# lebrice/blurred-GAN

Hardware: AMD Instinct MI355X
Metric: images/sec (G+D+GP step) (higher is better)
Workload: dtype f32; 1 GPU; celeba64 64x64x3 batch 256/GPU, blur sigma 5.0 (31 taps), D-step+GP+G-step+Adam; global_batch=256, parallelism=dp1

## Files before the change

blurred-gan_amd/_lib.py:

```python
from __future__ import annotations

import ctypes as C
import os

HERE = os.path.dirname(os.path.abspath(__file__))
LIB_PATH = os.environ.get("BGAN_HIP_LIB") or os.path.join(HERE, "libbgan_hip.so")


class BgError(RuntimeError):
    pass


class Epilogue(C.Structure):
    _fields_ = [("mode", C.c_int), ("bias", C.c_void_p), ("ref", C.c_void_p), ("keep", C.c_void_p),
                ("alpha", C.c_float), ("scale", C.c_float), ("splitk_ws", C.c_void_p), ("splitk_ws_bytes", C.c_size_t),
                ("keep_elems", C.c_size_t), ("stats", C.c_void_p), ("stats_capacity", C.c_size_t), ("stats_rows", C.POINTER(C.c_int))]


ABI_VERSION = 5
EPI_NONE, EPI_BIAS_LRELU, EPI_MUL_GRAD, EPI_TANH, EPI_AFFINE_LRELU = 0, 1, 2, 3, 4

_p, _i, _f, _z, _u64 = C.c_void_p, C.c_int, C.c_float, C.c_size_t, C.c_uint64

SIGNATURES = {
# ... 4 lines not shown
    "bg_prof_reset": (_i, []),
    "bg_prof_count": (_i, []),
    "bg_prof_get": (_i, [_i, C.c_char_p, _i, C.POINTER(_f), C.POINTER(C.c_double), C.POINTER(C.c_double)]),
    "bg_prof_get_exec": (_i, [_i, C.POINTER(C.c_double)]),
    "bg_prof_get_useful": (_i, [_i, C.POINTER(C.c_double)]),
    "bg_conv2d_useful_flops": (C.c_double, [_i] * 7),
    "bg_range_enable": (_i, [_i]),
    "bg_range_push": (_i, [C.c_char_p]),
    "bg_range_pop": (_i, []),
    "bg_blur_policy": (_i, [_f, _i, _i, C.POINTER(_f), C.POINTER(_f), C.POINTER(_i)]),
    "bg_gauss_kernel_1d": (_i, [_f, _f, C.POINTER(_f), _i, C.POINTER(_i)]),
    "bg_blur_workspace_bytes": (_z, [_i, _i, _i, _i, _i]),
    "bg_blur_nhwc_f32": (_i, [_p, _p, _i, _i, _i, _i, _p, _i, _p, _p]),
    "bg_blur3_lerp_supported": (_i, [_i, _i, _i, _i, _i]),
    "bg_blur3_lerp_nhwc_f32": (_i, [_p, _p, _p, _p, _i, _i, _i, _i, _p, _i, _p]),
    "bg_conv2d_splitk_workspace_bytes": (_z, [_i, _i, _i, _i, _i, _i, _i, _i]),
    "bg_conv2d_fwd": (_i, [_p, _p, _p, _i, _i, _i, _i, _i, _i, _i, C.POINTER(Epilogue), _p]),
    "bg_conv2d_bwd_data": (_i, [_p, _p, _p, _i, _i, _i, _i, _i, _i, _i, C.POINTER(Epilogue), _p]),
    "bg_conv2d_fwd_math": (_i, [_p, _p, _p, _i, _i, _i, _i, _i, _i, _i, C.POINTER(Epilogue), _p, _i]),
    "bg_conv2d_bwd_data_math": (_i, [_p, _p, _p, _i, _i, _i, _i, _i, _i, _i, C.POINTER(Epilogue), _p, _i]),
    "bg_conv2d_math_taken": (_i, [_i] * 9),
    "bg_conv2d_bwd_filter_workspace_bytes": (_z, [_i, _i, _i, _i, _i, _i, _i]),
    "bg_conv2d_bwd_filter": (_i, [_p, _p, _p, _i, _i, _i, _i, _i, _i, _i, _f, _f, _p, _z, _p]),
    "bg_transpose_last2": (_i, [_p, _p, _i, _i, _i, _p]),
    "bg_transpose_last2_batched": (_i, [_p, _p, _p, _i, _i, _p]),
    "bg_gemm_f32": (_i, [_p, _p, _p, _i, _i, _i, _i, _i, _p, _f, _f, _p]),
    "bg_colsum_workspace_bytes": (_z, [_i, _i]),
    "bg_colsum_f32": (_i, [_p, _p, _i, _i, _i, _f, _f, _p, _z, _p]),
    "bg_bn_workspace_bytes": (_z, [_i, _i]),
    "bg_bn_train_fwd": (_i, [_p, _p, _i, _i, _p, _p, _p, _p, _p, _p, _f, _f, _i, _f, _p, _z, _p]),
    "bg_bn_train_fwd_partials": (_i, [_p, _i, _p, _p, _i, _i, _p, _p, _p, _p, _p, _p, _f, _f, _i, _f, _p]),
    "bg_bn_sums_from_partials": (_i, [_p, _i, _i, _p, _p]),
    "bg_bn_infer_fwd": (_i, [_p, _p, _i, _i, _p, _p, _p, _p, _f, _f, _p]),
    "bg_bn_train_bwd": (_i, [_p, _p, _p, _p, _i, _i, _p, _p, _p, _p, _p, _p, _f, _p, _z, _p]),
    "bg_bn_fold_f32": (_i, [_p, _p, _p, _p, _f, _i, _p, _p, _p]),
    "bg_bn_fold_many_f32": (_i, [_i, _p, _p, _p, _p, _p, _p, _p, _p, _p]),
    "bg_bn_stats_f32": (_i, [_p, _i, _i, _p, _p, _z, _p]),
    "bg_bn_finalize_f32": (_i, [_p, _i, _i, _p, _p, _p, _p, _f, _f, _i, _p]),
    "bg_bn_apply_f32": (_i, [_p, _p, _i, _i, _p, _p, _p, _p, _f, _p]),
    "bg_bn_finalize_apply_f32": (_i, [_p, _i, _p, _p, _i, _i, _p, _p, _p, _p, _p, _p, _f, _f, _i, _f, _p]),
    "bg_bn_bwd_stats_f32": (_i, [_p, _p, _p, _i, _i, _p, _p, _p, _p, _f, _p, _p, _z, _p]),
    "bg_bn_bwd_apply_f32": (_i, [_p, _p, _p, _p, _i, _i, _i, _p, _p, _p, _p, _p, _f, _p]),
    "bg_bn_param_grads_f32": (_i, [_p, _i, _f, _p, _p, _p]),
    "bg_lerp_f32": (_i, [_p, _p, _p, _p, _i, _i, _p]),
    "bg_row_norm_f32": (_i, [_p, _p, _i, _i, _p]),
    "bg_gp_seed_f32": (_i, [_p, _p, _f, _p, _i, _i, _p]),
# ... 79 lines not shown
```

blurred-gan_amd/csrc/conv_wgrad.hip:

```cpp
#include "conv_common.h"
#include <algorithm>
#include <cmath>
#include <cstdlib>
#include <mutex>
#include <type_traits>
#include <utility>

namespace {

typedef float floatx16 __attribute__((ext_vector_type(16)));

struct WgradParams {
  const float* X;
  const float* DY;
  float* out;
  int B, H, W, Ci, Ho, Wo, Co;
  int k, s, pt, pl;
  int M;
  int chunk;
  int ksplit;
  int tiles_m, tiles_n, xcd_swizzle;
  float beta, scale;
  unsigned x_bytes, dy_bytes;
  unsigned mul_hw, sh_hw, mul_w, sh_w;
  int lg_w, lg_h, lg_b, pow2;
  int order_n;
  unsigned char tap_order[32];
};

__device__ inline int fastdiv(int m, unsigned mul, unsigned sh) { return (int)(((unsigned long long)(unsigned)m * mul) >> sh); }

template <int BM, int BN, int BKP, int WAVES_M, int WAVES_N, int WAVES_K, int P2>
__global__ __launch_bounds__(256) void conv_wgrad_v3_kernel(const WgradParams p) {
  static_assert(WAVES_M * WAVES_N * WAVES_K == 4, "4 waves");
  constexpr int WTM = BM / WAVES_M, WTN = BN / WAVES_N;
  constexpr int MI = WTM / 32, NI = WTN / 32;
  static_assert(MI >= 1 && NI >= 1 && WTM % 32 == 0 && WTN % 32 == 0, "wave tile");
  constexpr int TPR_A = BM / 4, RPP_A = 256 / TPR_A, AP = BKP / RPP_A;
  constexpr int TPR_B = BN / 4, RPP_B = 256 / TPR_B, BP = BKP / RPP_B;
  static_assert(AP >= 1 && BP >= 1 && BKP % RPP_A == 0 && BKP % RPP_B == 0, "loader passes must tile the chunk exactly");
  constexpr int STAGE = BKP * (BM + BN);
  constexpr int RED = (WAVES_K > 1) ? (WAVES_K - 1) * WAVES_M * WAVES_N * MI * NI * 1024 : 0;
  constexpr int SMEM = (2 * STAGE > RED) ? 2 * STAGE : RED;
  constexpr unsigned kOob = 0x80000000u;
  __shared__ __attribute__((aligned(16))) float smem[SMEM];

  const int tid = threadIdx.x, lane = tid & 63, wave = tid >> 6;
  const int wk = wave % WAVES_K, wmn = wave / WAVES_K;
  const int wm = wmn / WAVES_N, wn = wmn % WAVES_N;
  const int ntile = p.tiles_m * p.tiles_n, ntap = p.k * p.k;
  int tile, tap, zsplit;
  if (P2 == 2 && p.order_n > 0) {
    const int w = blockIdx.x, r = w >> 8;
    const int u = ((r & 1) && ((r + 1) << 8) <= (int)gridDim.x) ? (r << 8) + ((31 - ((w & 255) >> 3)) << 3) + (w & 7) : w;
    tile = u % ntile;
    const int rest = u / ntile;
    zsplit = rest % p.ksplit;
    tap = p.tap_order[rest / p.ksplit];
  } else {
    const int L = p.xcd_swizzle ? bg::xcd_remap(blockIdx.x, gridDim.x) : (int)blockIdx.x;
    tile = L % ntile; tap = (L / ntile) % ntap; zsplit = L / (ntile * ntap);
  }
  const int tile_m = tile / p.tiles_n, tile_n = tile % p.tiles_n;
  const int ci0 = tile_m * BM, co0 = tile_n * BN;
  const int kh = tap / p.k, kw = tap % p.k;
  const int m_begin = zsplit * p.chunk;
  const int m_end = min(p.M, m_begin + p.chunk);
  const int nsteps = (m_end - m_begin + BKP - 1) / BKP;

  const __amdgpu_buffer_rsrc_t rsX = __builtin_amdgcn_make_buffer_rsrc(const_cast<float*>(p.X), 0, (int)p.x_bytes, 0x00020000);
  const __amdgpu_buffer_rsrc_t rsY = __builtin_amdgcn_make_buffer_rsrc(const_cast<float*>(p.DY), 0, (int)p.dy_bytes, 0x00020000);
  const int arow = tid / TPR_A, aq = tid % TPR_A;
  const int brow = tid / TPR_B, bq = tid % TPR_B;
  const int HoWo = p.Ho * p.Wo;
  const bool a_col_ok = ci0 + aq * 4 < p.Ci, b_col_ok = co0 + bq * 4 < p.Co;
  const int a_coloff = (ci0 + aq * 4) * 4, b_coloff = (co0 + bq * 4) * 4;
  const int dyk = kh - p.pt, dxk = kw - p.pl;
  float4 regA[AP], regB[BP];

  const int WoS = p.Wo * p.s, HoS = p.Ho * p.s;
  int dstep_ow, dstep_oh, dstep_b;
// ... 39 lines not shown
      const int bb = r >> (p.lg_w + p.lg_h), oh = (r >> p.lg_w) & (p.Ho - 1), ow = r & (p.Wo - 1);
      t_r[i] = r;
      t_oy[i] = oh * p.s;
      t_ox[i] = ow * p.s;
      t_off[i] = (unsigned)(((bb * p.H + oh * p.s) * p.W + ow * p.s) * p.Ci * 4 + a_coloff);
    }
  }
  if (P2 == 2) {
#pragma unroll
    for (int i = 0; i < AP; ++i) {
      const int r = arow + i * RPP_A;
      t_r[i] = r;
      t_oy[i] = 0;
      t_ox[i] = 0;
      t_off[i] = a_col_ok ? (unsigned)(r * p.H * p.W * p.Ci * 4 + a_coloff) : kOob;
    }
#pragma unroll
    for (int i = 0; i < BP; ++i) b_off[i] = b_col_ok ? (unsigned)((brow + i * RPP_B) * HoWo * p.Co * 4 + b_coloff) : kOob;
  }
  int s_m0 = m_begin;
  int q_oh = 0, q_ow = 0, q_bc = 0, q_left = 0, q_ow_lo = 0, q_ow_hi = 0, q_nb = 1;
  int nsteps_live = 0;
  if (P2 == 2) {
    const int oh_lo = max(0, (-dyk + p.s - 1) / p.s), oh_hi = min(p.Ho - 1, (p.H - 1 - dyk) / p.s);
    const int ow_lo = max(0, (-dxk + p.s - 1) / p.s), ow_hi = min(p.Wo - 1, (p.W - 1 - dxk) / p.s);
    const int rh = max(0, oh_hi - oh_lo + 1), rw = max(0, ow_hi - ow_lo + 1);
    q_nb = p.B / BKP;
    const int nlive = rh * rw * q_nb;
    const int cpz = (nlive + p.ksplit - 1) / p.ksplit;
    const int q_begin = min(nlive, zsplit * cpz), q_end = min(nlive, q_begin + cpz);
    nsteps_live = q_end - q_begin;
    q_left = nsteps_live;
    const int pi = q_begin / q_nb;
    q_bc = q_begin - pi * q_nb;
    q_oh = oh_lo + (rw > 0 ? pi / rw : 0);
    q_ow = ow_lo + (rw > 0 ? pi % rw : 0);
    q_ow_lo = ow_lo; q_ow_hi = ow_hi;
  }

  auto gload = [&](int) {
    if (P2 == 2) {
      if (q_left > 0) {
        const int b0 = q_bc * BKP, pos = q_oh * p.Wo + q_ow;
        const unsigned offS = (unsigned)(((b0 * p.H + q_oh * p.s + dyk) * p.W + q_ow * p.s + dxk) * p.Ci * 4);
        const unsigned offY = (unsigned)((b0 * HoWo + pos) * p.Co * 4);
#pragma unroll
        for (int i = 0; i < AP; ++i)
          regA[i] = __builtin_bit_cast(float4, __builtin_amdgcn_raw_buffer_load_b128(rsX, t_off[i], (int)offS, 0));
#pragma unroll
        for (int i = 0; i < BP; ++i)
          regB[i] = __builtin_bit_cast(float4, __builtin_amdgcn_raw_buffer_load_b128(rsY, b_off[i], (int)offY, 0));
        --q_left;
        if (++q_bc == q_nb) {
// ... 113 lines not shown
    if (wk > 0) {
      float* red = smem + (((wk - 1) * WAVES_M * WAVES_N + wmn) * MI * NI) * 1024;
#pragma unroll
      for (int i = 0; i < MI; ++i)
#pragma unroll
        for (int j = 0; j < NI; ++j)
#pragma unroll
          for (int r = 0; r < 16; ++r) red[((i * NI + j) * 16 + r) * 64 + lane] = acc[i][j][r];
    }
    __syncthreads();
    if (wk > 0) return;
#pragma unroll
    for (int w = 1; w < WAVES_K; ++w) {
      const float* red = smem + (((w - 1) * WAVES_M * WAVES_N + wmn) * MI * NI) * 1024;
#pragma unroll
      for (int i = 0; i < MI; ++i)
#pragma unroll
        for (int j = 0; j < NI; ++j)
#pragma unroll
          for (int r = 0; r < 16; ++r) acc[i][j][r] += red[((i * NI + j) * 16 + r) * 64 + lane];
    }
  }

  float* out = p.out + (size_t)zsplit * p.k * p.k * p.Ci * p.Co + (size_t)tap * p.Ci * p.Co;
  const bool direct = p.ksplit == 1;
#pragma unroll
  for (int i = 0; i < MI; ++i)
#pragma unroll
    for (int j = 0; j < NI; ++j) {
      const int co = co0 + wn * WTN + j * 32 + (lane & 31);
#pragma unroll
      for (int r = 0; r < 16; ++r) {
        const int ci = ci0 + wm * WTM + i * 32 + (r & 3) + 8 * (r >> 2) + 4 * (lane >> 5);
        if (ci < p.Ci && co < p.Co) {
          float* q = out + (size_t)ci * p.Co + co;
          const float v = acc[i][j][r];
          if (direct) *q = (p.beta != 0.f ? p.beta * *q : 0.f) + p.scale * v;
          else *q = v;
        }
      }
    }
}

template <int TG, int BN, int WAVES_N, int WAVES_K>
__global__ __launch_bounds__(256) void conv_wgrad_tg_kernel(const WgradParams p) {
  static_assert(WAVES_N * WAVES_K == 4 && BN == 32 * WAVES_N, "one 32-wide co tile per wave column");
  constexpr int BKP = 32, BMc = 32, BM = TG * BMc;
  constexpr int TPR_B = BN / 4, RPP_B = 256 / TPR_B, BP = BKP / RPP_B;
// ... 1013 lines not shown
      red[zg][c] = make_float4(a.x + b.x, a.y + b.y, a.z + b.z, a.w + b.w);
    }
    __syncthreads();
  }
  if (zg != 0 || e >= n) return;
  const float4 a = red[0][c];
  float4 o = make_float4(scale * a.x, scale * a.y, scale * a.z, scale * a.w);
  if (beta != 0.f) {
    const float4 q = *reinterpret_cast<const float4*>(dw + e);
    o.x += beta * q.x; o.y += beta * q.y; o.z += beta * q.z; o.w += beta * q.w;
  }
  *reinterpret_cast<float4*>(dw + e) = o;
}

__global__ __launch_bounds__(256) void wgrad_reduce_scalar_kernel(const float* __restrict__ slabs, float* __restrict__ dw, int n,
                                                                  int ksplit, float beta, float scale) {
  const int e = blockIdx.x * 256 + threadIdx.x;
  if (e >= n) return;
  float s = 0.f;
  for (int z = 0; z < ksplit; ++z) s += slabs[(size_t)z * n + e];
  dw[e] = (beta != 0.f ? beta * dw[e] : 0.f) + scale * s;
}

struct WgradPlan {
  int mode;
  int ksplit, chunk, tiles_m, tiles_n, bkp, taps_in_grid;
  int always_slab;
};

inline bool strip_ok(int H, int W, int Ci, int Co, int k, int s) {
  if (k != 5 || s != 2 || (H & 1) || (W & 1) || Ci % 32 || Co % 64) return false;
  const int Wo = W / 2, Ho = H / 2;
  if (Wo != 8 && Wo != 16 && Wo != 32) return false;
  return Ho % (64 / Wo) == 0;
}

constexpr size_t kRowLdsMax = 64 * 1024;
inline int thin_ci_rows(int s) { return s == 2 ? 8 : 16; }
inline size_t thin_ci_lds(int W, int Ci, int Co, int k, int s) {
  return std::max((size_t)((thin_ci_rows(s) - 1) * s + k) * ((size_t)W * Ci + 2 * kTiHalo), (size_t)k * (Co / 16) * 4 * 64) * sizeof(float);
}
inline size_t thin_co_lds(int W, int Ci, int Co, int k) {
  return std::max((size_t)(kTcRows + k - 1) * ((size_t)W * Co + 2 * kTcHalo), (size_t)4 * k * (Ci / 16) * 4 * 64) * sizeof(float);
}

WgradPlan plan_wgrad(int B, int H, int W, int Ci, int Co, int k, int s) {
  WgradPlan pl{};
  int Ho, Wo, pt, pp;
  bg::same_pads(H, k, s, &Ho, &pt);
  bg::same_pads(W, k, s, &Wo, &pp);
  const long M = (long)B * Ho * Wo;
  const bool mfma = (Ci % 4 == 0) && (Co % 4 == 0) && Ci >= 16 && Co >= 16;
  const int kk = k * k;
  const bool thin_ci = Ci <= 4 && Co % 4 == 0 && Co >= 16 && kk * Ci <= 128;
  const bool thin_co = Co <= 4 && Ci % 4 == 0 && Ci >= 16 && s == 1 && kk * Co <= 128;
  int bm = 0, bn = 0;
  if (!mfma && !thin_ci && !thin_co) {
    pl.mode = 0;
    const long nblk = bg::cdiv((size_t)k * k * Ci * Co, 256);
    long want = std::max(1L, 2048 / nblk);
    long chunk = std::max(256L, (M + want - 1) / want);
    pl.chunk = (int)chunk;
    pl.ksplit = (int)((M + chunk - 1) / chunk);
    return pl;
  }
  static const int no_strip = getenv("BG_WGRAD_NO_STRIP") ? 1 : 0;
// ... 94 lines not shown
    want = std::max(1L, (tgt + base - 1) / base);
    want = std::min(want, std::max(1L, steps / (skipping ? 8 : 4)));
    if ((size_t)kk * Ci * Co * sizeof(float) > (8u << 20)) want = std::min(want, 2L);
  } else {
    const int bm_eff = pl.taps_in_grid == 2 ? k * bm : bm;
    const int lds = 2 * pl.bkp * (bm_eff + bn) * 4;
    const int per_cu = std::max(1, std::min(160 * 1024 / lds, 5));
    const double slots = 256.0 * per_cu;
    const double t_step = 2.0 * bm_eff * bn * pl.bkp * per_cu / 614e9 * 1e6;
    const double ovh = 5.0 / t_step;
    const double nout_bytes = (double)kk * Ci * Co * 4.0;
    double best = 1e30;
    want = 1;
    for (long ks = 1; ks <= std::min<long>(64, std::max(1L, steps / 4)); ++ks) {
      const double rounds = std::ceil(base * ks / slots);
      const double per_wg = std::ceil((double)steps / ks);
      const double cost = rounds * (per_wg + ovh) * t_step + (ks > 1 ? 5.0 + (ks + 1) * nout_bytes / 3.5e6 + ks * nout_bytes / 5e6 : 0.0);
      if (cost < best * 0.999) { best = cost; want = ks; }
    }
  }
  long chunk = ((M + want - 1) / want + pl.bkp - 1) / pl.bkp * pl.bkp;
  pl.chunk = (int)chunk;
  pl.ksplit = (int)((M + chunk - 1) / chunk);
  return pl;
}

}

extern "C" {

size_t bg_conv2d_bwd_filter_workspace_bytes(int B, int H, int W, int Cin, int Cout, int ksize, int stride) {
  if (B <= 0 || H <= 0 || W <= 0 || Cin <= 0 || Cout <= 0 || ksize <= 0 || stride <= 0) return 0;
  WgradPlan pl = plan_wgrad(B, H, W, Cin, Cout, ksize, stride);
  if (pl.ksplit <= 1 && !pl.always_slab) return 0;
  return (size_t)pl.ksplit * ksize * ksize * Cin * Cout * sizeof(float);
}

int bg_conv2d_bwd_filter(const float* x, const float* dy, float* dw, int B, int H, int W, int Cin, int Cout, int ksize,
                         int stride, float beta, float scale, void* ws_d, size_t ws_bytes, void* stream) {
  BG_REQUIRE(x && dy && dw, BG_ERR_NULL, "bg_conv2d_bwd_filter: null pointer");
  BG_REQUIRE(B > 0 && H > 0 && W > 0 && Cin > 0 && Cout > 0, BG_ERR_BAD_SHAPE, "bg_conv2d_bwd_filter: B=%d H=%d W=%d Cin=%d Cout=%d", B, H, W, Cin, Cout);
  BG_REQUIRE(ksize >= 1 && (ksize & 1) && ksize * ksize <= bg::kMaxTaps, BG_ERR_UNSUPPORTED, "bg_conv2d_bwd_filter: kernel size %d", ksize);
  BG_REQUIRE(stride == 1 || stride == 2, BG_ERR_UNSUPPORTED, "bg_conv2d_bwd_filter: stride %d", stride);
  BG_REQUIRE(bg::aligned16(x) && bg::aligned16(dy) && bg::aligned16(dw), BG_ERR_BAD_ALIGNMENT, "bg_conv2d_bwd_filter: pointers must be 16-byte aligned");
  bg::UsefulScope useful(bg::conv_useful_flops(B, H, W, Cin, Cout, ksize, stride));
  WgradPlan pl = plan_wgrad(B, H, W, Cin, Cout, ksize, stride);
  const size_t nout = (size_t)ksize * ksize * Cin * Cout;
  const bool slabs = pl.ksplit > 1 || pl.always_slab;
  const size_t need = slabs ? (size_t)pl.ksplit * nout * sizeof(float) : 0;
  BG_REQUIRE(need == 0 || (ws_d && ws_bytes >= need), BG_ERR_WORKSPACE, "bg_conv2d_bwd_filter: workspace %zu bytes < %zu needed", ws_bytes, need);
  WgradParams p;
  memset(&p, 0, sizeof p);
  p.X = x; p.DY = dy;
  p.B = B; p.H = H; p.W = W; p.Ci = Cin; p.Co = Cout; p.k = ksize; p.s = stride;
  bg::same_pads(H, ksize, stride, &p.Ho, &p.pt);
  bg::same_pads(W, ksize, stride, &p.Wo, &p.pl);
  p.M = B * p.Ho * p.Wo;
  BG_REQUIRE((size_t)B * H * W * (size_t)Cin < (1ull << 29) && (size_t)p.M * (size_t)Cout < (1ull << 29), BG_ERR_UNSUPPORTED,
             "bg_conv2d_bwd_filter: tensor exceeds 2 GiB");
  {
    auto magic = [](unsigned d, unsigned* mul, unsigned* sh) {
      unsigned sft = 0;
      while ((1ull << sft) < d) ++sft;
      *mul = (unsigned)((1ull << (31 + sft)) / d + 1);
      *sh = 31 + sft;
    };
    magic((unsigned)(p.Ho * p.Wo), &p.mul_hw, &p.sh_hw);
    magic((unsigned)p.Wo, &p.mul_w, &p.sh_w);
    auto lg2 = [](int v) { int l = 0; while ((1 << l) < v) ++l; return l; };
    p.lg_w = lg2(p.Wo); p.lg_h = lg2(p.Ho);
    p.pow2 = ((1 << p.lg_w) == p.Wo && (1 << p.lg_h) == p.Ho) ? 1 : 0;
    p.lg_b = lg2(B);
    static const int no_pm = getenv("BG_NO_POS_MAJOR") ? 1 : 0;
    if (p.pow2 && !no_pm && B % 128 == 0 && B >= 128 && p.Ho * p.Wo <= 16) p.pow2 = 2;
    p.x_bytes = (unsigned)((size_t)B * H * W * Cin * sizeof(float));
    p.dy_bytes = (unsigned)((size_t)p.M * Cout * sizeof(float));
  }
  p.chunk = pl.chunk; p.ksplit = pl.ksplit; p.tiles_n = pl.tiles_n; p.tiles_m = pl.tiles_m;
  {
    static const int swz = getenv("BG_WGRAD_SWZ") ? atoi(getenv("BG_WGRAD_SWZ")) : 0;
    static const int swz_tg = getenv("BG_WGRAD_SWZ_TG") ? atoi(getenv("BG_WGRAD_SWZ_TG")) : 1;
    p.xcd_swizzle = (pl.mode == 6 || pl.mode == 7) ? swz_tg : swz;
  }
  p.beta = beta; p.scale = scale;
  p.order_n = 0;
  {
    static const int no_sort = getenv("BG_NO_TILE_SORT") ? 1 : 0;
    if (p.pow2 == 2 && pl.taps_in_grid == 1 && pl.mode >= 1 && pl.mode <= 5 && !no_sort && ksize * ksize <= 32) {
      int live[32], idx[32];
      for (int t = 0; t < ksize * ksize; ++t) {
        const int dyk = t / ksize - p.pt, dxk = t % ksize - p.pl;
        auto floordiv = [](int a, int b) { return a >= 0 ? a / b : -((-a + b - 1) / b); };
        const int oh_lo = std::max(0, (-dyk + stride - 1) / stride), oh_hi = std::min(p.Ho - 1, floordiv(H - 1 - dyk, stride));
        const int ow_lo = std::max(0, (-dxk + stride - 1) / stride), ow_hi = std::min(p.Wo - 1, floordiv(W - 1 - dxk, stride));
        live[t] = std::max(0, oh_hi - oh_lo + 1) * std::max(0, ow_hi - ow_lo + 1);
        idx[t] = t;
      }
      std::stable_sort(idx, idx + ksize * ksize, [&](int a, int b) { return live[a] > live[b]; });
      for (int t = 0; t < ksize * ksize; ++t) p.tap_order[t] = (unsigned char)idx[t];
      p.order_n = ksize * ksize;
    }
  }
  p.out = slabs ? static_cast<float*>(ws_d) : dw;
  const double flops = 2.0 * p.M * (double)nout;
  const double abytes = 4.0 * ((double)B * H * W * Cin + (double)p.M * Cout + (double)nout * (beta != 0.f ? 2 : 1));
  int rc;
  if (pl.mode == 0) {
    bg::Launch L(stream, "conv_wgrad_direct", flops, abytes);
    bg::launch(wgrad_direct_kernel, dim3(bg::cdiv(nout, 256), pl.ksplit), dim3(256), 0, L.s, p);
    rc = L.done("wgrad_direct_kernel");
  } else if (pl.mode == 33) {
    bg::Launch L(stream, "conv_wgrad_mfma", flops, abytes);
    const int lgwo = p.Wo == 32 ? 5 : (p.Wo == 16 ? 4 : 3);
    const int spi = p.Ho / (64 / p.Wo), nstrips = B * spi, ntile = pl.tiles_m * pl.tiles_n;
    BG_LDS_ATTR_ONCE_V(conv_wgrad_strip_kernel<5>, StripGeom<5>::lds_bytes);
    BG_LDS_ATTR_ONCE_V(conv_wgrad_strip_kernel<4>, StripGeom<4>::lds_bytes);
    BG_LDS_ATTR_ONCE_V(conv_wgrad_strip_kernel<3>, StripGeom<3>::lds_bytes);
    const dim3 grid((unsigned)(ntile * pl.ksplit));
    if (lgwo == 5) bg::launch((conv_wgrad_strip_kernel<5>), grid, dim3(256), StripGeom<5>::lds_bytes, L.s, p, nstrips, spi, pl.chunk, ntile);
    else if (lgwo == 4) bg::launch((conv_wgrad_strip_kernel<4>), grid, dim3(256), StripGeom<4>::lds_bytes, L.s, p, nstrips, spi, pl.chunk, ntile);
    else bg::launch((conv_wgrad_strip_kernel<3>), grid, dim3(256), StripGeom<3>::lds_bytes, L.s, p, nstrips, spi, pl.chunk, ntile);
    rc = L.done("conv_wgrad_strip_kernel");
  } else if (pl.mode == 32) {
// ... 11 lines not shown
    const int bpi = (int)bg::cdiv(p.Ho, rb), nblocks = B * bpi;
    const int nt = Cout / 16;
    const size_t lds = thin_ci_lds(W, Cin, Cout, ksize, stride);
    BG_REQUIRE(lds <= kRowLdsMax, BG_ERR_UNSUPPORTED, "bg_conv2d_bwd_filter: thin-Ci row kernel needs %zu bytes of LDS", lds);
#define BG_TI(NTv, Kv) bg::launch((conv_wgrad_thin_ci_kernel<NTv, Kv>), dim3(pl.ksplit), dim3(256), lds, L.s, p, nblocks, bpi, rb)
    if (ksize == 5) { if (nt == 1) BG_TI(1, 5); else if (nt == 2) BG_TI(2, 5); else BG_TI(4, 5); }
    else { if (nt == 1) BG_TI(1, 3); else if (nt == 2) BG_TI(2, 3); else BG_TI(4, 3); }
#undef BG_TI
    rc = L.done("conv_wgrad_thin_ci_kernel");
  } else if (pl.mode == 30) {
    bg::Launch L(stream, "conv_wgrad_mfma_thin_co", flops, abytes);
    const int bpi = (int)bg::cdiv(H, kTcRows), nblocks = B * bpi;
    const int mt = Cin / 16;
    const size_t lds = thin_co_lds(W, Cin, Cout, ksize);
    BG_REQUIRE(lds <= kRowLdsMax, BG_ERR_UNSUPPORTED, "bg_conv2d_bwd_filter: thin-Co row kernel needs %zu bytes of LDS", lds);
    if (ksize == 5 && mt == 2) bg::launch((conv_wgrad_thin_co_kernel<2, 5>), dim3(pl.ksplit), dim3(256), lds, L.s, p, nblocks, bpi);
    else if (ksize == 5) bg::launch((conv_wgrad_thin_co_kernel<1, 5>), dim3(pl.ksplit), dim3(256), lds, L.s, p, nblocks, bpi);
    else if (mt == 2) bg::launch((conv_wgrad_thin_co_kernel<2, 3>), dim3(pl.ksplit), dim3(256), lds, L.s, p, nblocks, bpi);
    else bg::launch((conv_wgrad_thin_co_kernel<1, 3>), dim3(pl.ksplit), dim3(256), lds, L.s, p, nblocks, bpi);
    rc = L.done("conv_wgrad_thin_co_kernel");
  } else {
    dim3 grid(pl.tiles_m * pl.tiles_n, pl.taps_in_grid == 1 ? ksize * ksize : (pl.taps_in_grid == 2 ? ksize : 1), pl.ksplit);
    bg::Launch L(stream, pl.mode >= 20 ? "conv_wgrad_mfma_thin_co" : (pl.mode >= 10 ? "conv_wgrad_mfma_thin_ci" : "conv_wgrad_mfma"), flops, abytes);
    const dim3 grid1((unsigned)(grid.x * grid.y * grid.z));
    switch (pl.mode) {
#define BG_V3(BMv, BNv, BKv, WMv, WNv, WKv)                                                                               \
  do {                                                                                                                   \
    if (p.pow2 == 2) bg::launch((conv_wgrad_v3_kernel<BMv, BNv, BKv, WMv, WNv, WKv, 2>), grid1, dim3(256), 0, L.s, p);     \
    else if (p.pow2 == 1) bg::launch((conv_wgrad_v3_kernel<BMv, BNv, BKv, WMv, WNv, WKv, 1>), grid1, dim3(256), 0, L.s, p); \
    else bg::launch((conv_wgrad_v3_kernel<BMv, BNv, BKv, WMv, WNv, WKv, 0>), grid1, dim3(256), 0, L.s, p);        \
  } while (0)
      case 1: BG_V3(128, 128, 32, 2, 2, 1); break;
      case 2: BG_V3(64, 64, 32, 2, 2, 1); break;
      case 3: BG_V3(64, 32, 64, 2, 1, 2); break;
      case 4: BG_V3(32, 64, 64, 1, 2, 2); break;
      case 5: BG_V3(32, 32, 128, 1, 1, 4); break;
#undef BG_V3
      case 6: bg::launch((conv_wgrad_tg_kernel<5, 64, 2, 2>), grid1, dim3(256), 0, L.s, p); break;
      case 7: bg::launch((conv_wgrad_tg_kernel<5, 32, 1, 4>), grid1, dim3(256), 0, L.s, p); break;
      case 10: bg::launch((conv_wgrad_kernel<32, 64, 64, 1, 2, 2, 1>), grid, dim3(256), 0, L.s, p); break;
      case 11: bg::launch((conv_wgrad_kernel<96, 32, 64, 1, 1, 4, 1>), grid, dim3(256), 0, L.s, p); break;
      case 12: bg::launch((conv_wgrad_kernel<128, 32, 64, 1, 1, 4, 1>), grid, dim3(256), 0, L.s, p); break;
      case 20: bg::launch((conv_wgrad_kernel<64, 32, 64, 2, 1, 2, 2>), grid, dim3(256), 0, L.s, p); break;
      case 21: bg::launch((conv_wgrad_kernel<32, 96, 64, 1, 1, 4, 2>), grid, dim3(256), 0, L.s, p); break;
      default: bg::launch((conv_wgrad_kernel<32, 128, 64, 1, 1, 4, 2>), grid, dim3(256), 0, L.s, p); break;
    }
    rc = L.done("conv_wgrad_kernel");
  }
  if (rc) return rc;
  if (slabs) {
    bg::Launch L(stream, "conv_wgrad_reduce", 0, (double)(pl.ksplit + 1) * nout * 4);
    if (nout % 4 == 0 && bg::aligned16(ws_d) && pl.ksplit >= 64 && nout <= 65536)
      bg::launch(wgrad_reduce_tall_kernel, dim3(bg::cdiv(nout / 4, 16)), dim3(1024), 0, L.s, static_cast<const float*>(ws_d), dw,
                         (int)nout, pl.ksplit, beta, scale);
    else if (nout % 4 == 0 && bg::aligned16(ws_d))
      bg::launch(wgrad_reduce_kernel, dim3(bg::cdiv(nout / 4, 64)), dim3(256), 0, L.s, static_cast<const float*>(ws_d), dw,
                         (int)nout, pl.ksplit, beta, scale);
    else
      bg::launch(wgrad_reduce_scalar_kernel, dim3(bg::cdiv(nout, 256)), dim3(256), 0, L.s, static_cast<const float*>(ws_d), dw,
                         (int)nout, pl.ksplit, beta, scale);
    rc = L.done("wgrad_reduce_kernel");
  }
  return rc;
}

}
```

blurred-gan_amd/ops.py:

```python
from __future__ import annotations

import ctypes as C

import torch

from . import _lib, program
from ._lib import Epilogue, EPI_NONE, EPI_BIAS_LRELU, EPI_MUL_GRAD, EPI_TANH, EPI_AFFINE_LRELU, check

LRELU_ALPHA = 0.3


_dev_index = None
_raw_stream = getattr(torch._C, "_cuda_getCurrentRawStream", None)
_get_device = getattr(torch._C, "_cuda_getDevice", None)


def _stream():
    if _raw_stream is None or _get_device is None:
        return C.c_void_p(torch.cuda.current_stream().cuda_stream)
    cur = _get_device()
    if _dev_index is not None and cur != _dev_index:
        raise BgDeviceError(f"operands live on cuda:{_dev_index} but the current device is cuda:{cur}")
    return _raw_stream(cur)

# ... 122 lines not shown


def conv2d_bwd_data(dy, w, dx, ksize, stride, epi=None, math="fp32"):
    code = conv_math_code(math)
    _f32(dy, w, dx)
    B, H, W, Cin = dx.shape
    Cout = dy.shape[3]
    assert w.numel() == ksize * ksize * Cin * Cout
    assert tuple(dy.shape) == (B, same_out(H, stride), same_out(W, stride), Cout), (dy.shape, dx.shape)
    e = C.byref(epi) if epi is not None else None
    if code == 0:
        check(_lib.load().bg_conv2d_bwd_data(_ptr(dy), _ptr(w), _ptr(dx), B, H, W, Cin, Cout, ksize, stride, e, _stream()),
              "bg_conv2d_bwd_data")
    else:
        check(_lib.load().bg_conv2d_bwd_data_math(_ptr(dy), _ptr(w), _ptr(dx), B, H, W, Cin, Cout, ksize, stride, e, _stream(), code),
              "bg_conv2d_bwd_data_math")
    return dx


def conv2d_bwd_filter_workspace_bytes(B, H, W, Cin, Cout, ksize, stride):
    return _lib.load().bg_conv2d_bwd_filter_workspace_bytes(B, H, W, Cin, Cout, ksize, stride)


def conv2d_bwd_filter(x, dy, dw, ksize, stride, beta=0.0, scale=1.0, ws=None):
    _f32(x, dy, dw)
    B, H, W, Cin = x.shape
    Cout = dy.shape[3]
    assert dw.numel() == ksize * ksize * Cin * Cout
    assert tuple(dy.shape[:3]) == (B, same_out(H, stride), same_out(W, stride))
    wsb = ws.numel() * ws.element_size() if ws is not None else 0
    check(_lib.load().bg_conv2d_bwd_filter(_ptr(x), _ptr(dy), _ptr(dw), B, H, W, Cin, Cout, ksize, stride, beta, scale,
                                           _ptr(ws), wsb, _stream()), "bg_conv2d_bwd_filter")
    return dw


def transpose_last2(src, dst, T, R, Cc):
    _f32(src, dst)
    assert src.numel() == T * R * Cc == dst.numel()
    check(_lib.load().bg_transpose_last2(_ptr(src), _ptr(dst), T, R, Cc, _stream()), "bg_transpose_last2")
    return dst


def transpose_last2_batched(src_base, dst_base, desc, n, total_tiles):
    _f32(src_base, dst_base)
    assert desc.dtype == torch.int32 and desc.is_contiguous() and desc.numel() == 6 * n
    check(_lib.load().bg_transpose_last2_batched(_ptr(src_base), _ptr(dst_base), _ptr(desc), n, total_tiles, _stream()),
# ... 393 lines not shown
```

include/bgan.h:

```cpp
#ifndef BGAN_H
#define BGAN_H

#include <stddef.h>
#include <stdint.h>

#ifdef __cplusplus
extern "C" {
#endif

#define BG_ABI_VERSION 5

typedef enum {
  BG_OK = 0,
  BG_ERR_BAD_SHAPE = -1,
  BG_ERR_BAD_ALIGNMENT = -2,
  BG_ERR_UNSUPPORTED = -3,
  BG_ERR_HIP = -4,
  BG_ERR_WORKSPACE = -5,
  BG_ERR_NULL = -6,
  BG_ERR_RCCL = -7
} bg_status;

int bg_version(void);
const char* bg_last_error(void);
// ... 38 lines not shown
  float scale;
  void* splitk_ws;
  size_t splitk_ws_bytes;
  size_t keep_elems;
  float* stats;
  size_t stats_capacity;
  int* stats_rows;
} bg_epilogue;

size_t bg_conv2d_splitk_workspace_bytes(int bwd_data, int B, int H, int W, int Cin, int Cout, int ksize, int stride);
int bg_conv2d_fwd(const float* x, const float* wT_d, float* y, int B, int H, int W, int Cin, int Cout,
                  int ksize, int stride, const bg_epilogue* epi, void* stream);
int bg_conv2d_bwd_data(const float* dy, const float* w_d, float* dx, int B, int H, int W, int Cin, int Cout,
                       int ksize, int stride, const bg_epilogue* epi, void* stream);
typedef enum { BG_CONV_MATH_FP32 = 0, BG_CONV_MATH_BF16X6 = 1 } bg_conv_math;
int bg_conv2d_fwd_math(const float* x, const float* wT_d, float* y, int B, int H, int W, int Cin, int Cout,
                       int ksize, int stride, const bg_epilogue* epi, void* stream, int math);
int bg_conv2d_bwd_data_math(const float* dy, const float* w_d, float* dx, int B, int H, int W, int Cin, int Cout,
                            int ksize, int stride, const bg_epilogue* epi, void* stream, int math);
int bg_conv2d_math_taken(int bwd_data, int B, int H, int W, int Cin, int Cout, int ksize, int stride, int math);
size_t bg_conv2d_bwd_filter_workspace_bytes(int B, int H, int W, int Cin, int Cout, int ksize, int stride);
int bg_conv2d_bwd_filter(const float* x, const float* dy, float* dw, int B, int H, int W, int Cin, int Cout,
                         int ksize, int stride, float beta, float scale, void* ws_d, size_t ws_bytes, void* stream);
int bg_transpose_last2(const float* src, float* dst, int T, int R, int C, void* stream);
int bg_transpose_last2_batched(const float* src_base, float* dst_base, const int* desc_d, int n, int total_tiles, void* stream);

int bg_gemm_f32(const float* A, const float* Bm, float* C, int M, int N, int K, int transA, int transB,
                const float* bias, float beta, float scale, void* stream);

size_t bg_colsum_workspace_bytes(int M, int N);
int bg_colsum_f32(const float* x, float* out, int M, int N, int square, float beta, float scale,
                  void* ws_d, size_t ws_bytes, void* stream);

size_t bg_bn_workspace_bytes(int M, int C);
int bg_bn_train_fwd(const float* x, float* y, int M, int C, const float* gamma, const float* beta,
                    float* moving_mean, float* moving_var, float* save_mean, float* save_inv,
                    float eps, float momentum, int unbiased, float lrelu_alpha,
                    void* ws_d, size_t ws_bytes, void* stream);
int bg_bn_infer_fwd(const float* x, float* y, int M, int C, const float* gamma, const float* beta,
                    const float* moving_mean, const float* moving_var, float eps, float lrelu_alpha, void* stream);
int bg_bn_train_bwd(const float* dy, const float* y, const float* x, float* dx, int M, int C,
                    const float* gamma, const float* beta, const float* save_mean, const float* save_inv,
                    float* dgamma, float* dbeta, float lrelu_alpha, void* ws_d, size_t ws_bytes, void* stream);

int bg_bn_fold_f32(const float* gamma, const float* beta, const float* moving_mean, const float* moving_var, float eps, int C,
                   float* scale_out, float* shift_out, void* stream);
// ... 102 lines not shown
```

Measured before the change: 32840 images/s.

## Balance wgrad split-K per tap by live positions using a simulated makespan planner

In the position-major wgrad path, each tap now gets its own number of K-splits, sized by how many output positions are live for that tap, in place of a uniform ksplit. A host-side planner simulates CU scheduling to choose the split counts and weighs that against the cost of writing and reducing the slabs. A new per-tap reduce kernel sums the variable-size slabs into dw. The aim is to even out work across blocks for small-spatial layers, where border taps have fewer live positions; the cost is more planning logic and a different workspace size.

```diff
diff --git a/blurred-gan_amd/_lib.py b/blurred-gan_amd/_lib.py
--- a/blurred-gan_amd/_lib.py
+++ b/blurred-gan_amd/_lib.py
@@ -50,6 +50,7 @@
     "bg_conv2d_math_taken": (_i, [_i] * 9),
     "bg_conv2d_bwd_filter_workspace_bytes": (_z, [_i, _i, _i, _i, _i, _i, _i]),
     "bg_conv2d_bwd_filter": (_i, [_p, _p, _p, _i, _i, _i, _i, _i, _i, _i, _f, _f, _p, _z, _p]),
+    "bg_conv2d_bwd_filter_plan": (_i, [_i] * 7 + [C.POINTER(_i), C.POINTER(_i), C.POINTER(_i), C.POINTER(_z)]),
     "bg_transpose_last2": (_i, [_p, _p, _i, _i, _i, _p]),
     "bg_transpose_last2_batched": (_i, [_p, _p, _p, _i, _i, _p]),
     "bg_gemm_f32": (_i, [_p, _p, _p, _i, _i, _i, _i, _i, _p, _f, _f, _p]),
diff --git a/blurred-gan_amd/csrc/conv_wgrad.hip b/blurred-gan_amd/csrc/conv_wgrad.hip
--- a/blurred-gan_amd/csrc/conv_wgrad.hip
+++ b/blurred-gan_amd/csrc/conv_wgrad.hip
@@ -2,7 +2,10 @@
 #include <algorithm>
 #include <cmath>
 #include <cstdlib>
+#include <cstring>
 #include <mutex>
+#include <queue>
+#include <vector>
 #include <type_traits>
 #include <utility>
 
@@ -26,6 +29,8 @@
   int lg_w, lg_h, lg_b, pow2;
   int order_n;
   unsigned char tap_order[32];
+  int pm_n;
+  unsigned short tap_nsplit[32], tap_nlong[32], unit_long[32], unit_short[32], tap_slab[32];
 };
 
 __device__ inline int fastdiv(int m, unsigned mul, unsigned sh) { return (int)(((unsigned long long)(unsigned)m * mul) >> sh); }
@@ -55,8 +60,17 @@
     const int u = ((r & 1) && ((r + 1) << 8) <= (int)gridDim.x) ? (r << 8) + ((31 - ((w & 255) >> 3)) << 3) + (w & 7) : w;
     tile = u % ntile;
     const int rest = u / ntile;
-    zsplit = rest % p.ksplit;
-    tap = p.tap_order[rest / p.ksplit];
+    if (p.pm_n > 0) {
+      tap = 0; zsplit = 0;
+      for (int t = 0; t < ntap; ++t) {
+        const int nl = p.tap_nlong[t], a = rest - p.unit_long[t], b = rest - p.unit_short[t];
+        if ((unsigned)a < (unsigned)nl) { tap = t; zsplit = a; }
+        if ((unsigned)b < (unsigned)(p.tap_nsplit[t] - nl)) { tap = t; zsplit = nl + b; }
+      }
+    } else {
+      zsplit = rest % p.ksplit;
+      tap = p.tap_order[rest / p.ksplit];
+    }
   } else {
     const int L = p.xcd_swizzle ? bg::xcd_remap(blockIdx.x, gridDim.x) : (int)blockIdx.x;
     tile = L % ntile; tap = (L / ntile) % ntap; zsplit = L / (ntile * ntap);
@@ -142,13 +156,22 @@
   int q_oh = 0, q_ow = 0, q_bc = 0, q_left = 0, q_ow_lo = 0, q_ow_hi = 0, q_nb = 1;
   int nsteps_live = 0;
   if (P2 == 2) {
-    const int oh_lo = max(0, (-dyk + p.s - 1) / p.s), oh_hi = min(p.Ho - 1, (p.H - 1 - dyk) / p.s);
-    const int ow_lo = max(0, (-dxk + p.s - 1) / p.s), ow_hi = min(p.Wo - 1, (p.W - 1 - dxk) / p.s);
+    auto floordiv = [](int a, int b) { return a >= 0 ? a / b : -((-a + b - 1) / b); };
+    const int oh_lo = max(0, (-dyk + p.s - 1) / p.s), oh_hi = min(p.Ho - 1, floordiv(p.H - 1 - dyk, p.s));
+    const int ow_lo = max(0, (-dxk + p.s - 1) / p.s), ow_hi = min(p.Wo - 1, floordiv(p.W - 1 - dxk, p.s));
     const int rh = max(0, oh_hi - oh_lo + 1), rw = max(0, ow_hi - ow_lo + 1);
     q_nb = p.B / BKP;
     const int nlive = rh * rw * q_nb;
-    const int cpz = (nlive + p.ksplit - 1) / p.ksplit;
-    const int q_begin = min(nlive, zsplit * cpz), q_end = min(nlive, q_begin + cpz);
+    int q_begin, q_end;
+    if (p.pm_n > 0) {
+      const int ns = p.tap_nsplit[tap], nl = p.tap_nlong[tap], cq = (nlive - nl) / ns;
+      q_begin = zsplit * cq + min(zsplit, nl);
+      q_end = q_begin + cq + (zsplit < nl ? 1 : 0);
+    } else {
+      const int cpz = (nlive + p.ksplit - 1) / p.ksplit;
+      q_begin = min(nlive, zsplit * cpz);
+      q_end = min(nlive, q_begin + cpz);
+    }
     nsteps_live = q_end - q_begin;
     q_left = nsteps_live;
     const int pi = q_begin / q_nb;
@@ -308,8 +331,10 @@
     }
   }
 
-  float* out = p.out + (size_t)zsplit * p.k * p.k * p.Ci * p.Co + (size_t)tap * p.Ci * p.Co;
-  const bool direct = p.ksplit == 1;
+  const bool pm_split = P2 == 2 && p.pm_n > 0;
+  float* out = pm_split ? p.out + (size_t)(p.tap_slab[tap] + zsplit) * p.Ci * p.Co
+                        : p.out + (size_t)zsplit * p.k * p.k * p.Ci * p.Co + (size_t)tap * p.Ci * p.Co;
+  const bool direct = p.ksplit == 1 && !pm_split;
 #pragma unroll
   for (int i = 0; i < MI; ++i)
 #pragma unroll
@@ -1369,10 +1394,59 @@
   dw[e] = (beta != 0.f ? beta * dw[e] : 0.f) + scale * s;
 }
 
+struct ReduceTaps {
+  unsigned short nsplit[32], slab[32];
+};
+
+template <int V>
+__global__ __launch_bounds__(256) void wgrad_reduce_taps_kernel(const float* __restrict__ slabs, float* __restrict__ dw, int n_tap,
+                                                                const ReduceTaps tb, float beta, float scale) {
+  const int tap = blockIdx.y;
+  const int e = (blockIdx.x * 256 + threadIdx.x) * V;
+  if (e >= n_tap) return;
+  const int ns = tb.nsplit[tap];
+  const float* src = slabs + (size_t)tb.slab[tap] * n_tap + e;
+  float* q = dw + (size_t)tap * n_tap + e;
+  if (V == 4) {
+    float4 s = make_float4(0.f, 0.f, 0.f, 0.f);
+    int z = 0;
+    for (; z + 4 <= ns; z += 4) {
+      float4 v[4];
+#pragma unroll
+      for (int i = 0; i < 4; ++i) v[i] = *reinterpret_cast<const float4*>(src + (size_t)(z + i) * n_tap);
+#pragma unroll
+      for (int i = 0; i < 4; ++i) { s.x += v[i].x; s.y += v[i].y; s.z += v[i].z; s.w += v[i].w; }
+    }
+    for (; z < ns; ++z) {
+      const float4 v = *reinterpret_cast<const float4*>(src + (size_t)z * n_tap);
+      s.x += v.x; s.y += v.y; s.z += v.z; s.w += v.w;
+    }
+    float4 o = make_float4(scale * s.x, scale * s.y, scale * s.z, scale * s.w);
+    if (beta != 0.f) {
+      const float4 d = *reinterpret_cast<const float4*>(q);
+      o.x += beta * d.x; o.y += beta * d.y; o.z += beta * d.z; o.w += beta * d.w;
+    }
+    *reinterpret_cast<float4*>(q) = o;
+  } else {
+    float s = 0.f;
+    for (int z = 0; z < ns; ++z) s += src[(size_t)z * n_tap];
+    float o = scale * s;
+    if (beta != 0.f) o += beta * *q;
+    *q = o;
+  }
+}
+
+struct PmSplit {
+  int n, nunits;
+  unsigned short nsplit[32], nlong[32], unit_long[32], unit_short[32], slab[32];
+};
+
 struct WgradPlan {
   int mode;
   int ksplit, chunk, tiles_m, tiles_n, bkp, taps_in_grid;
   int always_slab;
+  int pm;
+  PmSplit split;
 };
 
 inline bool strip_ok(int H, int W, int Ci, int Co, int k, int s) {
@@ -1389,6 +1463,165 @@
 }
 inline size_t thin_co_lds(int W, int Ci, int Co, int k) {
   return std::max((size_t)(kTcRows + k - 1) * ((size_t)W * Co + 2 * kTcHalo), (size_t)4 * k * (Ci / 16) * 4 * 64) * sizeof(float);
+}
+
+inline int live_positions(int H, int W, int Ho, int Wo, int pt, int pp, int k, int s, int t) {
+  const int dyk = t / k - pt, dxk = t % k - pp;
+  auto floordiv = [](int a, int b) { return a >= 0 ? a / b : -((-a + b - 1) / b); };
+  const int oh_lo = std::max(0, (-dyk + s - 1) / s), oh_hi = std::min(Ho - 1, floordiv(H - 1 - dyk, s));
+  const int ow_lo = std::max(0, (-dxk + s - 1) / s), ow_hi = std::min(Wo - 1, floordiv(W - 1 - dxk, s));
+  return std::max(0, oh_hi - oh_lo + 1) * std::max(0, ow_hi - ow_lo + 1);
+}
+
+inline bool pos_major_ok(int B, int Ho, int Wo) {
+  static const int no_pm = getenv("BG_NO_POS_MAJOR") ? 1 : 0;
+  return !no_pm && (Ho & (Ho - 1)) == 0 && (Wo & (Wo - 1)) == 0 && B % 128 == 0 && B >= 128 && Ho * Wo <= 16;
+}
+
+void pm_order(PmSplit& sp, const int* lc, std::vector<int>* len_out) {
+  int idx[32], q[32];
+  for (int t = 0; t < sp.n; ++t) {
+    idx[t] = t;
+    q[t] = lc[t] / sp.nsplit[t];
+    sp.nlong[t] = (unsigned short)(lc[t] % sp.nsplit[t]);
+  }
+  std::stable_sort(idx, idx + sp.n, [&](int a, int b) { return q[a] > q[b]; });
+  if (len_out) len_out->clear();
+  int u = 0, slab = 0;
+  for (int i = 0; i < sp.n;) {
+    int j = i;
+    while (j < sp.n && q[idx[j]] == q[idx[i]]) ++j;
+    for (int m = i; m < j; ++m) {
+      const int t = idx[m];
+      sp.unit_long[t] = (unsigned short)u;
+      u += sp.nlong[t];
+      if (len_out) len_out->insert(len_out->end(), sp.nlong[t], q[t] + 1);
+    }
+    for (int m = i; m < j; ++m) {
+      const int t = idx[m];
+      sp.unit_short[t] = (unsigned short)u;
+      u += sp.nsplit[t] - sp.nlong[t];
+      if (len_out) len_out->insert(len_out->end(), sp.nsplit[t] - sp.nlong[t], q[t]);
+    }
+    i = j;
+  }
+  for (int t = 0; t < sp.n; ++t) {
+    sp.slab[t] = (unsigned short)slab;
+    slab += sp.nsplit[t];
+  }
+  sp.nunits = slab;
+}
+
+double pm_makespan(const std::vector<int>& len, int ntile, int per_cu, double ovh) {
+  constexpr int ncu = 256;
+  const int N = (int)len.size() * ntile;
+  auto work = [&](int w) {
+    const int r = w >> 8;
+    const int u = ((r & 1) && ((r + 1) << 8) <= N) ? (r << 8) + ((31 - ((w & 255) >> 3)) << 3) + (w & 7) : w;
+    return (double)len[u / ntile] + ovh;
+  };
+  struct Cu { double T, V, v[8]; int r; };
+  std::vector<Cu> cu(ncu);
+  for (auto& c : cu) { c.T = c.V = 0.0; c.r = 0; }
+  auto next_done = [](const Cu& c) {
+    double m = c.v[0];
+    for (int i = 1; i < c.r; ++i) m = std::min(m, c.v[i]);
+    return c.T + (m - c.V) * (c.r == 1 ? 1.0 / 0.7 : (double)c.r);
+  };
+  typedef std::pair<double, int> Ev;
+  std::priority_queue<Ev, std::vector<Ev>, std::greater<Ev>> heap;
+  int next = 0;
+  for (; next < N && next < ncu * per_cu; ++next) {
+    Cu& c = cu[next % ncu];
+    c.v[c.r++] = work(next);
+  }
+  for (int i = 0; i < ncu; ++i)
+    if (cu[i].r) heap.push(Ev(next_done(cu[i]), i));
+  double end = 0.0;
+  while (!heap.empty()) {
+    const Ev ev = heap.top();
+    heap.pop();
+    Cu& c = cu[ev.second];
+    int mi = 0;
+    for (int i = 1; i < c.r; ++i)
+      if (c.v[i] < c.v[mi]) mi = i;
+    c.T = end = ev.first;
+    c.V = c.v[mi];
+    c.v[mi] = c.v[--c.r];
+    if (next < N) c.v[c.r++] = c.V + work(next++);
+    if (c.r) heap.push(Ev(next_done(c), ev.second));
+  }
+  return end;
+}
+
+PmSplit plan_pm_split(int B, int H, int W, int Ci, int Co, int k, int s, int bm, int bn, int bkp, int ntile, int ksplit_uniform) {
+  struct Key { int v[7]; };
+  static std::mutex mu;
+  static std::vector<std::pair<Key, PmSplit>> cache;
+  const Key key{{B, H, W, Ci, Co, k, s}};
+  {
+    std::lock_guard<std::mutex> g(mu);
+    for (const auto& e : cache)
+      if (!memcmp(&e.first, &key, sizeof key)) return e.second;
+  }
+  int Ho, Wo, pt, pp;
+  bg::same_pads(H, k, s, &Ho, &pt);
+  bg::same_pads(W, k, s, &Wo, &pp);
+  const int kk = k * k;
+  int lc[32], cap[32];
+  PmSplit sp{};
+  sp.n = kk;
+  for (int t = 0; t < kk; ++t) {
+    lc[t] = live_positions(H, W, Ho, Wo, pt, pp, k, s, t) * (B / bkp);
+    cap[t] = std::max(1, std::min(lc[t] / 4, 4096));
+    sp.nsplit[t] = 1;
+  }
+  const int lds = 2 * bkp * (bm + bn) * 4;
+  const int per_cu = std::max(1, std::min(160 * 1024 / lds, 5));
+  const double t_step = 2.0 * bm * bn * bkp / 614e9 * 1e6;
+  const double ovh = 5.0 / (t_step * per_cu);
+  const double tap_bytes = (double)Ci * Co * 4.0;
+  auto slab_cost = [&](int S) { return 5.0 + (S + kk) * tap_bytes / 3.5e6 + S * tap_bytes / 5e6; };
+  PmSplit best = sp;
+  double best_cost = 1e30;
+  std::vector<int> len;
+  int S = kk;
+  static const int tgt_env = getenv("BG_WGRAD_TARGET") ? atoi(getenv("BG_WGRAD_TARGET")) : 0;
+  for (;;) {
+    if (S % kk == 0) {
+      if (tgt_env) {
+        best = sp;
+        if (S * ntile >= tgt_env) break;
+      } else {
+        if (slab_cost(S) >= best_cost) break;
+        pm_order(sp, lc, &len);
+        const double cost = pm_makespan(len, ntile, per_cu, ovh) * t_step + slab_cost(S);
+        if (cost < best_cost * 0.999) { best_cost = cost; best = sp; }
+      }
+    }
+    int pick = -1;
+    for (int t = 0; t < kk; ++t)
+      if (sp.nsplit[t] < cap[t] && (pick < 0 || (long)lc[t] * sp.nsplit[pick] > (long)lc[pick] * sp.nsplit[t])) pick = t;
+    if (pick < 0 || (long)(S + 1) * ntile > 8192 || S + 1 > 2048) break;
+    ++sp.nsplit[pick];
+    ++S;
+  }
+  if (!tgt_env) {
+    int idx[32];
+    for (int t = 0; t < kk; ++t) idx[t] = t;
+    std::stable_sort(idx, idx + kk, [&](int a, int b) { return lc[a] > lc[b]; });
+    len.clear();
+    for (int i = 0; i < kk; ++i) {
+      const int l = lc[idx[i]], cpz = (l + ksplit_uniform - 1) / ksplit_uniform;
+      for (int z = 0; z < ksplit_uniform; ++z) len.push_back(std::min(l, (z + 1) * cpz) - std::min(l, z * cpz));
+    }
+    const double cost = pm_makespan(len, ntile, per_cu, ovh) * t_step + slab_cost(ksplit_uniform * kk);
+    if (ksplit_uniform > 1 && cost <= best_cost) best.n = 0;
+  }
+  if (best.n) pm_order(best, lc, nullptr);
+  std::lock_guard<std::mutex> g(mu);
+  cache.emplace_back(key, best);
+  return best;
 }
 
 WgradPlan plan_wgrad(int B, int H, int W, int Ci, int Co, int k, int s) {
@@ -1529,7 +1762,24 @@
   long chunk = ((M + want - 1) / want + pl.bkp - 1) / pl.bkp * pl.bkp;
   pl.chunk = (int)chunk;
   pl.ksplit = (int)((M + chunk - 1) / chunk);
+  pl.pm = pos_major_ok(B, Ho, Wo) ? 1 : 0;
+  static const int no_sort = getenv("BG_NO_TILE_SORT") ? 1 : 0;
+  static const int pm_uniform = (getenv("BG_WGRAD_PM_SPLIT") && !strcmp(getenv("BG_WGRAD_PM_SPLIT"), "uniform")) ? 1 : 0;
+  if (pl.pm && pl.taps_in_grid == 1 && pl.mode >= 1 && pl.mode <= 5 && !no_sort && kk <= 32 && !pm_uniform) {
+    pl.split = plan_pm_split(B, H, W, Ci, Co, k, s, bm, bn, pl.bkp, pl.tiles_m * pl.tiles_n, pl.ksplit);
+    if (pl.split.n) {
+      pl.always_slab = 1;
+      pl.ksplit = 0;
+      for (int t = 0; t < kk; ++t) pl.ksplit = std::max(pl.ksplit, (int)pl.split.nsplit[t]);
+    }
+  }
   return pl;
+}
+
+inline size_t plan_ws_bytes(const WgradPlan& pl, int Ci, int Co, int k) {
+  if (pl.split.n) return (size_t)pl.split.nunits * Ci * Co * sizeof(float);
+  if (pl.ksplit <= 1 && !pl.always_slab) return 0;
+  return (size_t)pl.ksplit * k * k * Ci * Co * sizeof(float);
 }
 
 }
@@ -1538,9 +1788,22 @@
 
 size_t bg_conv2d_bwd_filter_workspace_bytes(int B, int H, int W, int Cin, int Cout, int ksize, int stride) {
   if (B <= 0 || H <= 0 || W <= 0 || Cin <= 0 || Cout <= 0 || ksize <= 0 || stride <= 0) return 0;
-  WgradPlan pl = plan_wgrad(B, H, W, Cin, Cout, ksize, stride);
-  if (pl.ksplit <= 1 && !pl.always_slab) return 0;
-  return (size_t)pl.ksplit * ksize * ksize * Cin * Cout * sizeof(float);
+  return plan_ws_bytes(plan_wgrad(B, H, W, Cin, Cout, ksize, stride), Cin, Cout, ksize);
+}
+
+int bg_conv2d_bwd_filter_plan(int B, int H, int W, int Cin, int Cout, int ksize, int stride, int* mode, int* nunits, int* nsplit,
+                              size_t* ws_bytes) {
+  BG_REQUIRE(B > 0 && H > 0 && W > 0 && Cin > 0 && Cout > 0, BG_ERR_BAD_SHAPE, "bg_conv2d_bwd_filter_plan: B=%d H=%d W=%d Cin=%d Cout=%d", B, H, W, Cin, Cout);
+  BG_REQUIRE(ksize >= 1 && (ksize & 1) && ksize * ksize <= bg::kMaxTaps, BG_ERR_UNSUPPORTED, "bg_conv2d_bwd_filter_plan: kernel size %d", ksize);
+  BG_REQUIRE(stride == 1 || stride == 2, BG_ERR_UNSUPPORTED, "bg_conv2d_bwd_filter_plan: stride %d", stride);
+  const WgradPlan pl = plan_wgrad(B, H, W, Cin, Cout, ksize, stride);
+  const int kk = ksize * ksize;
+  if (mode) *mode = pl.mode;
+  if (nunits) *nunits = pl.split.n ? pl.split.nunits : pl.ksplit * kk;
+  if (nsplit)
+    for (int t = 0; t < 32; ++t) nsplit[t] = t >= kk ? 0 : (pl.split.n ? (int)pl.split.nsplit[t] : pl.ksplit);
+  if (ws_bytes) *ws_bytes = plan_ws_bytes(pl, Cin, Cout, ksize);
+  return BG_OK;
 }
 
 int bg_conv2d_bwd_filter(const float* x, const float* dy, float* dw, int B, int H, int W, int Cin, int Cout, int ksize,
@@ -1554,7 +1817,7 @@
   WgradPlan pl = plan_wgrad(B, H, W, Cin, Cout, ksize, stride);
   const size_t nout = (size_t)ksize * ksize * Cin * Cout;
   const bool slabs = pl.ksplit > 1 || pl.always_slab;
-  const size_t need = slabs ? (size_t)pl.ksplit * nout * sizeof(float) : 0;
+  const size_t need = plan_ws_bytes(pl, Cin, Cout, ksize);
   BG_REQUIRE(need == 0 || (ws_d && ws_bytes >= need), BG_ERR_WORKSPACE, "bg_conv2d_bwd_filter: workspace %zu bytes < %zu needed", ws_bytes, need);
   WgradParams p;
   memset(&p, 0, sizeof p);
@@ -1578,8 +1841,7 @@
     p.lg_w = lg2(p.Wo); p.lg_h = lg2(p.Ho);
     p.pow2 = ((1 << p.lg_w) == p.Wo && (1 << p.lg_h) == p.Ho) ? 1 : 0;
     p.lg_b = lg2(B);
-    static const int no_pm = getenv("BG_NO_POS_MAJOR") ? 1 : 0;
-    if (p.pow2 && !no_pm && B % 128 == 0 && B >= 128 && p.Ho * p.Wo <= 16) p.pow2 = 2;
+    if (p.pow2 && pos_major_ok(B, p.Ho, p.Wo)) p.pow2 = 2;
     p.x_bytes = (unsigned)((size_t)B * H * W * Cin * sizeof(float));
     p.dy_bytes = (unsigned)((size_t)p.M * Cout * sizeof(float));
   }
@@ -1596,16 +1858,20 @@
     if (p.pow2 == 2 && pl.taps_in_grid == 1 && pl.mode >= 1 && pl.mode <= 5 && !no_sort && ksize * ksize <= 32) {
       int live[32], idx[32];
       for (int t = 0; t < ksize * ksize; ++t) {
-        const int dyk = t / ksize - p.pt, dxk = t % ksize - p.pl;
-        auto floordiv = [](int a, int b) { return a >= 0 ? a / b : -((-a + b - 1) / b); };
-        const int oh_lo = std::max(0, (-dyk + stride - 1) / stride), oh_hi = std::min(p.Ho - 1, floordiv(H - 1 - dyk, stride));
-        const int ow_lo = std::max(0, (-dxk + stride - 1) / stride), ow_hi = std::min(p.Wo - 1, floordiv(W - 1 - dxk, stride));
-        live[t] = std::max(0, oh_hi - oh_lo + 1) * std::max(0, ow_hi - ow_lo + 1);
+        live[t] = live_positions(H, W, p.Ho, p.Wo, p.pt, p.pl, ksize, stride, t);
         idx[t] = t;
       }
       std::stable_sort(idx, idx + ksize * ksize, [&](int a, int b) { return live[a] > live[b]; });
       for (int t = 0; t < ksize * ksize; ++t) p.tap_order[t] = (unsigned char)idx[t];
       p.order_n = ksize * ksize;
+    }
+    if (pl.split.n) {
+      p.pm_n = pl.split.n;
+      memcpy(p.tap_nsplit, pl.split.nsplit, sizeof p.tap_nsplit);
+      memcpy(p.tap_nlong, pl.split.nlong, sizeof p.tap_nlong);
+      memcpy(p.unit_long, pl.split.unit_long, sizeof p.unit_long);
+      memcpy(p.unit_short, pl.split.unit_short, sizeof p.unit_short);
+      memcpy(p.tap_slab, pl.split.slab, sizeof p.tap_slab);
     }
   }
   p.out = slabs ? static_cast<float*>(ws_d) : dw;
@@ -1663,7 +1929,7 @@
   } else {
     dim3 grid(pl.tiles_m * pl.tiles_n, pl.taps_in_grid == 1 ? ksize * ksize : (pl.taps_in_grid == 2 ? ksize : 1), pl.ksplit);
     bg::Launch L(stream, pl.mode >= 20 ? "conv_wgrad_mfma_thin_co" : (pl.mode >= 10 ? "conv_wgrad_mfma_thin_ci" : "conv_wgrad_mfma"), flops, abytes);
-    const dim3 grid1((unsigned)(grid.x * grid.y * grid.z));
+    const dim3 grid1(pl.split.n ? (unsigned)(grid.x * pl.split.nunits) : (unsigned)(grid.x * grid.y * grid.z));
     switch (pl.mode) {
 #define BG_V3(BMv, BNv, BKv, WMv, WNv, WKv)                                                                               \
   do {                                                                                                                   \
@@ -1689,7 +1955,20 @@
     rc = L.done("conv_wgrad_kernel");
   }
   if (rc) return rc;
-  if (slabs) {
+  if (pl.split.n) {
+    const int n_tap = Cin * Cout;
+    bg::Launch L(stream, "conv_wgrad_reduce", 0, ((double)pl.split.nunits * n_tap + (double)nout) * 4);
+    ReduceTaps tb;
+    memcpy(tb.nsplit, pl.split.nsplit, sizeof tb.nsplit);
+    memcpy(tb.slab, pl.split.slab, sizeof tb.slab);
+    if (bg::aligned16(ws_d))
+      bg::launch(wgrad_reduce_taps_kernel<4>, dim3(bg::cdiv(n_tap / 4, 256), ksize * ksize), dim3(256), 0, L.s,
+                 static_cast<const float*>(ws_d), dw, n_tap, tb, beta, scale);
+    else
+      bg::launch(wgrad_reduce_taps_kernel<1>, dim3(bg::cdiv(n_tap, 256), ksize * ksize), dim3(256), 0, L.s,
+                 static_cast<const float*>(ws_d), dw, n_tap, tb, beta, scale);
+    rc = L.done("wgrad_reduce_taps_kernel");
+  } else if (slabs) {
     bg::Launch L(stream, "conv_wgrad_reduce", 0, (double)(pl.ksplit + 1) * nout * 4);
     if (nout % 4 == 0 && bg::aligned16(ws_d) && pl.ksplit >= 64 && nout <= 65536)
       bg::launch(wgrad_reduce_tall_kernel, dim3(bg::cdiv(nout / 4, 16)), dim3(1024), 0, L.s, static_cast<const float*>(ws_d), dw,
diff --git a/blurred-gan_amd/ops.py b/blurred-gan_amd/ops.py
--- a/blurred-gan_amd/ops.py
+++ b/blurred-gan_amd/ops.py
@@ -168,6 +168,14 @@
     return _lib.load().bg_conv2d_bwd_filter_workspace_bytes(B, H, W, Cin, Cout, ksize, stride)
 
 
+def conv2d_bwd_filter_plan(B, H, W, Cin, Cout, ksize, stride):
+    mode, nunits, wsb = C.c_int(), C.c_int(), C.c_size_t()
+    nsplit = (C.c_int * 32)()
+    check(_lib.load().bg_conv2d_bwd_filter_plan(B, H, W, Cin, Cout, ksize, stride, C.byref(mode), C.byref(nunits), nsplit, C.byref(wsb)),
+          "bg_conv2d_bwd_filter_plan")
+    return mode.value, nunits.value, list(nsplit[:ksize * ksize]), wsb.value
+
+
 def conv2d_bwd_filter(x, dy, dw, ksize, stride, beta=0.0, scale=1.0, ws=None):
     _f32(x, dy, dw)
     B, H, W, Cin = x.shape
diff --git a/include/bgan.h b/include/bgan.h
--- a/include/bgan.h
+++ b/include/bgan.h
@@ -84,6 +84,8 @@
 size_t bg_conv2d_bwd_filter_workspace_bytes(int B, int H, int W, int Cin, int Cout, int ksize, int stride);
 int bg_conv2d_bwd_filter(const float* x, const float* dy, float* dw, int B, int H, int W, int Cin, int Cout,
                          int ksize, int stride, float beta, float scale, void* ws_d, size_t ws_bytes, void* stream);
+int bg_conv2d_bwd_filter_plan(int B, int H, int W, int Cin, int Cout, int ksize, int stride, int* mode, int* nunits,
+                              int* nsplit, size_t* ws_bytes);
 int bg_transpose_last2(const float* src, float* dst, int T, int R, int C, void* stream);
 int bg_transpose_last2_batched(const float* src_base, float* dst_base, const int* desc_d, int n, int total_tiles, void* stream);
 
```

After: 33090 images/s, median of 6. Within noise of the previous version (+0.8%).
